# maxjiang93/space_time_pde

Measured on AMD Instinct MI355X. Metric: query-points/sec (fwd+PDE-residual bwd), rb2d 128^3 latent, higher is better.
Workload: dtype f32; 1 GPU; BASELINE configs[1]: latent [1,32,128,128,32], 2^20 query points, RB2 (3 transport + continuity), ImNet nf=32 softplus, L1 losses, backward to ImNet + UNet3d parameters; points=1048576, parallelism=points sharded x1, unet=UNet3d(igres=(32, 128, 128), nf=16, mf=256) fwd+bwd inside the timed step

## Files before the change

include/stpde_hip.h:

```cpp
#ifndef STPDE_HIP_H
#define STPDE_HIP_H

#ifdef __cplusplus
extern "C" {
#endif

#define STPDE_OK 0
#define STPDE_E_BADARG 1
#define STPDE_E_UNSUPPORTED 2
#define STPDE_E_LAUNCH 3

#define STPDE_ACT_TANH 0
#define STPDE_ACT_RELU 1
#define STPDE_ACT_SOFTPLUS 2
#define STPDE_ACT_ELU 3
#define STPDE_ACT_SWISH 4
#define STPDE_ACT_LEAKYRELU 5

#define STPDE_XT 3
#define STPDE_PBAR_SLOTS 64

typedef struct {
  int S1;
  int S2;
  int pair0[6];
  int pair1[6];
  int act;
  float act_param;
  int combo;
  float alpha[6];
} stpde_jet_cfg;

int stpde_version(void);
int stpde_last_error(char* buf, unsigned long n);
#define STPDE_TUNE_CONV3_LDS_OFF 0
#define STPDE_TUNE_CONV3_LDS_MINBLK 1
#define STPDE_TUNE_CONV3_LDS_GX 2
#define STPDE_TUNE_CONV_WGRAD_LDS_GX 3
#define STPDE_TUNE_CONV1_WGRAD_LDS_GX 4
#define STPDE_TUNE_COUNT 5
int stpde_tune(const char* name, int value);
int stpde_trace_enable(int on);
long stpde_trace_read(char* buf, unsigned long n);

typedef struct {
  int P, N, B, n0, n1, n2, C;
  int p_base;
  float lo_c[3], hi_c[3], cube[3];
  float alpha[6];
} stpde_gather_desc;
int stpde_lig_gather(const stpde_gather_desc* d, const float* pts, const float* latent, float* X, float* XR,
                     float* coef, int* cell, float* cw , void* stream);

typedef struct {
  int ntiles, KT, MT, first_hidden;
  stpde_jet_cfg cfg;
  int mfma_bf16;
  int packed;
  int det;
} stpde_layer_desc;
int stpde_jet_layer_fwd(const stpde_layer_desc* d, const float* in_pre, const float* X, const float* Wh_pack,
                        const float* Ws_pack, const float* tanc, const float* W0s_pack, const float* tanc0,
                        float* out_pre, const float* cw ,
                        const void* Wh_pack_bf16, float* z0, void* stream);

int stpde_jet_tail_fwd(const stpde_jet_cfg* cfg, int ntiles, int nf16, const float* in_pre2, const float* X,
                       const float* const* Wh_pack, const float* const* Ws_pack, const float* const* tanc,
                       float* const* out_pre, const float* cw, void* stream);

int stpde_jet_tail_fwd_p(const stpde_jet_cfg* cfg, int ntiles, int nf16, const float* in_pre2, const float* X,
                         const float* const* Wh_pack, const float* const* Ws_pack, const float* const* tanc,
                         float* const* out_pre, const float* cw, int packed, const void* const* Wh16_pack, void* stream);

int stpde_jet_tail_bwd(const stpde_jet_cfg* cfg, int ntiles, int nf16, const float* abar5, const float* const* WhT_pack,
                       const float* const* pre, float* const* abar_out, const float* cw, float* act_param_bar,
                       void* stream);

int stpde_jet_tail_bwd_p(const stpde_jet_cfg* cfg, int ntiles, int nf16, const float* abar5, const float* const* WhT_pack,
                         const float* const* pre, float* const* abar_out, const float* cw, float* act_param_bar, int packed,
                         const void* const* WhT16_pack, void* stream);

int stpde_jet_layer_bwd(const stpde_layer_desc* d, const float* abar_out, const float* WhT_pack, float* in_pre,
                        const float* X, const float* W0s_pack, const float* tanc0, float* abar0, const float* cw,
                        float* act_param_bar, const void* WhT_pack_bf16 ,
                        float* abar0_tan, const float* z0, void* stream);

int stpde_jet_layer_bwd_to(const stpde_layer_desc* d, const float* abar_out, const float* WhT_pack, const float* in_pre,
                           float* abar_in, const float* cw, float* act_param_bar, const void* WhT_pack_bf16, void* stream);

int stpde_jet_wgrad(const stpde_layer_desc* d, int SP, const float* abar_out, const float* in_pre, const float* X,
                    const float* tanc0, float* dW_aug, const float* cw, void* stream);

int stpde_jet_fc1_bwd_supported(const stpde_layer_desc* d);
int stpde_jet_fc1_bwd(const stpde_layer_desc* d, const float* abar1, const void* WhT_pack_bf16, const float* z0,
                      const float* tanc0, const float* cw, const float* X, float* abar0, float* abar0_tan, float* dW_aug,
                      float* act_param_bar, void* stream);

int stpde_lig_reduce_fwd(const stpde_jet_cfg* cfg, int S_mlp, int P, int n_out, const float* out_pre,
                         const float* coef, float* jets, long ldp, void* stream);
int stpde_lig_reduce_bwd(const stpde_jet_cfg* cfg, int S_mlp, int P, int n_out, const float* jets_bar, long ldp,
                         const float* coef, float* abar_out, void* stream);

int stpde_jet_tan0_reduce(int ntiles, int MT, const float* abar0_tan, float* dW_aug, int ldw, int det ,
                          void* stream);

typedef struct {
  int ntiles, nlayers, C, n1, n2;
  int MT[8];
  int SP[8];
  int packed[8];
  int S[8];
} stpde_xbar_desc;
int stpde_lig_xbar_scatter(const stpde_xbar_desc* d, const float* const* abar, const float* const* WsL_pack,
                           const int* cell, float* dlatent, void* stream);
int stpde_lig_xbar_rows(const stpde_xbar_desc* d, const float* const* abar, const float* const* WsL_pack,
                        float* xrows, void* stream);
int stpde_lig_dlatent_reduce(int B, int n0, int n1, int n2, int C, const float* xrows, const int* perm,
                             const int* start, float* dlatent, void* stream);

typedef struct {
  int nlayers;
  int cin, cout, nf16;
  int KT[8], MT[8];
  const float* Wh[8];
  const float* WhT[8];
  const float* Ws[8];
  const float* WsL[8];
  const float* tanc[8];
  const void* Wh16[8];
  const void* WhT16[8];
  int mfma_bf16;
  int packed_mask;
  long dw_off[8];
} stpde_imnet_plan;
typedef struct {
  float* X;
  float* XR;
  float* coef;
  float* cw;
  int* cell;
  float* pre[8];
  float* abar2x;
  float* abar3x;
  float* tan0;
  float* abar0;
  float* abar1x;
  float* abar0x;
  float* xrows;
  int* perm;
  int* start;
  void* sort_tmp;
  unsigned long sort_tmp_bytes;
  float* abar4x;
} stpde_lig_workspace;
#define STPDE_F_STASH 1
#define STPDE_F_VALUE_TILES 2
#define STPDE_F_FUSED_TAIL 4
#define STPDE_F_TAN0_ROWSUM 8
#define STPDE_F_DETERMINISTIC 16
#define STPDE_F_WGRAD 32
#define STPDE_F_WGRAD_FP32 64
#define STPDE_F_PHASE_A 128
#define STPDE_F_PHASE_B 256
#define STPDE_F_NO_FC1_FUSED 512
#define STPDE_F_DET 1024
int stpde_lig_imnet_jet_fwd(const stpde_imnet_plan* plan, const stpde_jet_cfg* cfg_mlp, const stpde_jet_cfg* cfg_out,
                            const stpde_gather_desc* gd, const float* pts, const float* latent,
                            const stpde_lig_workspace* ws, float* jets, long ldp, int flags, void* stream);
int stpde_lig_imnet_jet_bwd(const stpde_imnet_plan* plan, const stpde_jet_cfg* cfg_mlp, const stpde_jet_cfg* cfg_out,
                            const stpde_jet_cfg* cfg_val, const stpde_gather_desc* gd, const stpde_lig_workspace* ws,
                            const float* jets_bar, long ldp, float* dW_flat, float* dlatent, float* act_param_bar,
                            int flags, void* stream);
unsigned long stpde_lig_sort_tmp_bytes(int P, long n_nodes);
int stpde_lig_cell_sort(int P, long n_nodes, const int* cell, int* perm, int* start, void* tmp, unsigned long tmp_bytes,
                        void* stream);

typedef struct {
  int P, N, B, dim, C;
  int n[4];
  float lo_c[4], hi_c[4], cube[4];
} stpde_interp_desc;
int stpde_interp_fwd(const stpde_interp_desc* d, const float* grid, const float* pts, float* out ,
                     float* corner_values , float* weights ,
                     float* x_relative , void* stream);
int stpde_interp_bwd_grid(const stpde_interp_desc* d, const float* pts, const float* out_bar,
                          const float* corner_bar, float* dgrid, void* stream);

typedef struct {
  int B, T, Z, X, Ci, Co, ksize;
  int det;
  int mfma_bf16;
} stpde_conv3d_desc;
#define STPDE_DET_K 6
int stpde_det_finalize(const void* acc, long n, float* out, void* stream);
int stpde_conv3d_fwd(const stpde_conv3d_desc* d, const float* x, const float* w_pack, const float* bias, float* y,
                     void* stream);
int stpde_conv3d_wgrad(const stpde_conv3d_desc* d, const float* x, const float* ybar, float* dW, void* stream);
int stpde_conv3d_wgrad_bias(const stpde_conv3d_desc* d, const float* x, const float* ybar, float* dW, float* dbias,
                            void* stream);

typedef struct {
  stpde_conv3d_desc d;
  const float* x;
  const float* w_pack;
  const float* bias;
  float* y;
  const float* x2;
  const float* w2_pack;
  float* y2;
  const float* wo2_pack;
  const float* bias2;
  const double* in_sums;
  const float* in_gamma;
  const float* in_beta;
  float* in_running_mean;
  float* in_running_var;
  float* in_stat;
  double* out_sums;
  const float* m;
  const float* m_stat;
  const float* m_gamma;
  const float* m_beta;
  float* m_bsum;
  int Ci2, Co2;
  float in_eps, in_momentum;
} stpde_conv3d_fused_args;
int stpde_conv3d_fused(const stpde_conv3d_fused_args* a, int* epilogue_done, void* stream);
int stpde_conv3d_wgrad_onload(const stpde_conv3d_desc* d, const float* x, const float* ybar, float* dW, float* dbias,
                              const float* in_stat, const float* in_gamma, const float* in_beta, void* stream);

#define STPDE_BN_REP 16
typedef struct {
  long N;
  int C, training, relu;
  float eps, momentum;
  int scratch_zeroed;
  int stats_mode;
  int reduce_done;
  int det;
} stpde_bn_desc;
int stpde_bn_fwd(const stpde_bn_desc* d, const float* x, const float* residual, const float* gamma, const float* beta,
                 float* running_mean, float* running_var, float* sums, float* stat, float* y, void* stream);
int stpde_bn_bwd(const stpde_bn_desc* d, const float* x, const float* y, const float* dy, const float* gamma,
                 const float* stat, float* bsum, float* dx, float* dresidual, float* dgamma, float* dbeta, void* stream);

typedef struct {
  int B, T, Z, X, C, ft, fz, fx;
} stpde_resample_desc;
int stpde_resample3d(const stpde_resample_desc* d, int mode, const float* in, const float* aux, float* out,
                     void* stream);

#define STPDE_RES_MAX_INS 192
enum {
  STPDE_RES_JET = 0, STPDE_RES_X, STPDE_RES_CONST, STPDE_RES_ADD, STPDE_RES_SUB, STPDE_RES_MUL, STPDE_RES_DIV,
  STPDE_RES_NEG, STPDE_RES_POWI, STPDE_RES_SIN, STPDE_RES_COS, STPDE_RES_EXP, STPDE_RES_LOG, STPDE_RES_SQRT,
  STPDE_RES_TANH, STPDE_RES_ABS, STPDE_RES_OUT
};
typedef struct {
  int op, a, b;
  float c;
} stpde_res_ins;
int stpde_residual_fwd(const stpde_res_ins* prog_dev, int nins, int n_eq, int n_out, int P, const float* jets,
                       long ld_stream, long ld_channel, const float* x , float* res, void* stream);
int stpde_residual_bwd(const stpde_res_ins* prog_dev, int nins, int n_eq, int n_out, int P, const float* jets,
                       long ld_stream, long ld_channel, const float* x, const float* res_bar, float* jets_bar,
                       void* stream);

#define STPDE_LOSS_L1 0
#define STPDE_LOSS_L2 1
#define STPDE_LOSS_HUBER 2
#define STPDE_LOSS_DET 16
int stpde_loss_sum(int kind, long n, const float* a, const float* b, float* out_sum, void* stream);
int stpde_loss_grad(int kind, long n, const float* a, const float* b, const float* grad_sum_dev, float* grad_a,
                    void* stream);

typedef struct {
  long n;
  float clip, beta1, beta2, eps, weight_decay, step_size, bias2_sqrt;
} stpde_adam_desc;
int stpde_clip_adam(const stpde_adam_desc* d, float* param, const float* grad, float* exp_avg, float* exp_avg_sq,
                    void* stream);
typedef struct {
  float* p;
  const float* g;
  float* m;
  float* v;
  long n;
  float step_size, bias2_sqrt;
} stpde_adam_tensor;
typedef struct {
  int tensor, pad;
  long offset;
} stpde_adam_chunk;
int stpde_clip_adam_multi(const stpde_adam_desc* d, const stpde_adam_tensor* tensors_dev,
                          const stpde_adam_chunk* chunks_dev, int nchunks, int chunk_elems, void* stream);

#ifdef __cplusplus
}
#endif
#endif
```

space_time_pde_amd/csrc/api.cpp:

```cpp
#include <hip/hip_runtime.h>

#include <cstdarg>
#include <cstdio>
#include <cstring>
#include <mutex>
#include <set>
#include <string>

#include "../../include/stpde_hip.h"

static thread_local char g_err[512] = "";

void stpde_set_error(const char* fmt, ...) {
  va_list ap;
  va_start(ap, fmt);
  vsnprintf(g_err, sizeof(g_err), fmt, ap);
  va_end(ap);
}

int stpde_check_launch(const char* what) {
  hipError_t e = hipGetLastError();
  if (e != hipSuccess) {
    stpde_set_error("%s: launch failed: %s", what, hipGetErrorString(e));
    return STPDE_E_LAUNCH;
  }
  return STPDE_OK;
}

extern "C" int stpde_version(void) { return 315; }

#include <atomic>
static const char* const g_tune_names[STPDE_TUNE_COUNT] = {"conv3_lds_off", "conv3_lds_minblk", "conv3_lds_gx", "conv_wgrad_lds_gx",
                                                           "conv1_wgrad_lds_gx"};
static std::atomic<int> g_tune[STPDE_TUNE_COUNT];
int stpde_tune_get(int key) { return (key >= 0 && key < STPDE_TUNE_COUNT) ? g_tune[key].load(std::memory_order_relaxed) : 0; }
extern "C" int stpde_tune(const char* name, int value) {
  if (!name) return -1;
  for (int k = 0; k < STPDE_TUNE_COUNT; ++k)
    if (!strcmp(name, g_tune_names[k])) return g_tune[k].exchange(value);
  stpde_set_error("stpde_tune: unknown key '%s'", name);
  return -1;
}

extern "C" int stpde_last_error(char* buf, unsigned long n) {
  if (!buf || n == 0) return STPDE_E_BADARG;
  strncpy(buf, g_err, n - 1);
  buf[n - 1] = 0;
  return STPDE_OK;
}

int stpde_trace_on = 0;
static std::mutex g_trace_mu;
static std::set<std::string> g_trace;

void stpde_trace_note(const char* launcher, const char* kernel) {
  std::lock_guard<std::mutex> lk(g_trace_mu);
  g_trace.insert(std::string(kernel) + " @ " + launcher);
}

extern "C" int stpde_trace_enable(int on) {
  std::lock_guard<std::mutex> lk(g_trace_mu);
  g_trace.clear();
  stpde_trace_on = on ? 1 : 0;
  return STPDE_OK;
}

extern "C" long stpde_trace_read(char* buf, unsigned long n) {
  std::lock_guard<std::mutex> lk(g_trace_mu);
  std::string all;
  for (const auto& s : g_trace) all += s + "\n";
  if (buf && n > 0) {
    strncpy(buf, all.c_str(), n - 1);
    buf[n - 1] = 0;
  }
  return (long)all.size() + 1;
}
```

space_time_pde_amd/csrc/jet_layer_impl.h:

```cpp
#pragma once
#include <cstdlib>

#include "common.h"

enum { PRO_NONE = 0, PRO_ACT = 1, PRO_L0 = 2 };
enum { EPI_FWD = 0, EPI_ADJ = 1, EPI_ADJ_L0 = 2 };
#ifndef STPDE_ABLATE
#define STPDE_ABLATE 0
#endif

#ifndef STPDE_STAMP
#define STPDE_STAMP 0
#endif
#ifndef STPDE_FWD2_OCC3
#define STPDE_FWD2_OCC3 1
#endif
#ifndef STPDE_FWD2_OCC_N
#define STPDE_FWD2_OCC_N 3
#endif
#ifndef STPDE_EARLY_L0
#define STPDE_EARLY_L0 1
#endif
#ifndef STPDE_EPI_PF
#define STPDE_EPI_PF 1
#endif
#ifndef STPDE_EPI_PF_BF
#define STPDE_EPI_PF_BF 1
#endif
#ifndef STPDE_EPI_PF_DEPTH
#define STPDE_EPI_PF_DEPTH 1
#endif
#ifndef STPDE_EPI_OPF
#define STPDE_EPI_OPF 3
#endif
#ifndef STPDE_X3_STREAM_OUTER
#define STPDE_X3_STREAM_OUTER 1
#endif
#ifndef STPDE_X3_EARLY
#define STPDE_X3_EARLY 0
#endif
#ifndef STPDE_X3_Z0P
#define STPDE_X3_Z0P 0
#endif
#ifndef STPDE_SKIP_FIRST_BAR
#define STPDE_SKIP_FIRST_BAR 1
#endif
#if STPDE_STAMP
#define STPDE_STAMP_B0 8192
static __device__ unsigned long long g_stamp[256 * 8 * 16];
#define STAMP(i)                                                                                          \
  do {                                                                                                    \
    if (blockIdx.x >= STPDE_STAMP_B0 && blockIdx.x < STPDE_STAMP_B0 + 256 && (threadIdx.x & 63) == 0)     \
      g_stamp[((blockIdx.x - STPDE_STAMP_B0) * 8 + (threadIdx.x >> 6)) * 16 + (i)] = __builtin_readcyclecounter(); \
  } while (0)
#else
#define STAMP(i)
#endif

struct LayerArgs {
  const float* Bin;
  const float* Wp;
  const float* X;
  const float* W0s;
  const float* tanc0;
  const float* Wsp;
  const float* tanc;
  float* Out;
  const float* Pre;
  const float* cw;
  const void* Wp16;
  int nsplit;
  float* pbar;
  float* Tan0;
  float* Z0;
  int KT, MT, ntiles;
  int split;
  int pk;
  stpde_jet_cfg cfg;
};

__device__ __forceinline__ f32x4 layer0_block(const float* W0s, int nblk, int blk, int lo, const f32x4* xb) {
  f32x4 part[XT];
#pragma unroll
  for (int xt = 0; xt < XT; ++xt) {
    f32x4 w = ld4x(W0s + ((size_t)xt * nblk + blk) * 256 + lo, xt);
    f32x4 c = f32x4{0.f, 0.f, 0.f, 0.f};
#pragma unroll
    for (int r = 0; r < x_live(xt); ++r) c = mfma4(w[r], xb[xt][r], c);
    part[xt] = c;
  }
  return (part[0] + part[1]) + part[2];
}

template <int S1, int S2, int EPI, int ACT, int PKM = 0>
__device__ __forceinline__ void layer_epilogue(const LayerArgs& a, int tile, int mt, int MT, int lane, f32x4* accm,
                                               const f32x4 (*xbv)[XT], const float* cq, float& pacc,
                                               const f32x4* z0pre = nullptr, const f32x4* prepf = nullptr,
                                               const f32x4* wspf = nullptr, const f32x4* tcpf = nullptr) {
  constexpr int S = 1 + S1 + S2;
  constexpr bool VT = S1 == 0 && S2 > 0;
  const int lo = lane * 4;
  f32x4 (&acc)[1][S] = *reinterpret_cast<f32x4 (*)[1][S]>(accm);
  constexpr int mi = 0;
    if (EPI == EPI_FWD) {
#pragma unroll
      for (int xt = 0; xt < XT; ++xt) {
        f32x4 w = wspf ? wspf[xt] : ld4x(a.Wsp + ((size_t)xt * MT + mt) * 256 + lo, xt);
#pragma unroll
        for (int sv = 0; sv < (VT ? S : 1); ++sv)
#pragma unroll
          for (int r = 0; r < x_live(xt); ++r) acc[mi][sv] = mfma4(w[r], xbv[sv][xt][r], acc[mi][sv]);
      }
      if (S1 == 3) {
#pragma unroll
        for (int d = 0; d < 3; ++d) acc[mi][1 + d] += tcpf ? tcpf[d] : ld4(a.tanc + ((size_t)d * MT + mt) * 256 + lo);
      }
#pragma unroll
      for (int st = 0; st < S; ++st) st_blk(a.Out, (PKM & 2) ? 1 : 0, tile, S, MT, st, mt, lane, acc[mi][st]);
    } else {
      f32x4 pre[S], ab[S];
      if (EPI == EPI_ADJ) {
#pragma unroll
        for (int st = 0; st < S; ++st)
          pre[st] = prepf ? prepf[st] : ld_blk(a.Pre, (PKM & 4) ? 1 : 0, tile, S, MT, st, mt, lane);
      } else {
        pre[0] = z0pre ? *z0pre : ld4(a.Z0 + ((size_t)tile * MT + mt) * 256 + lo);
        if (S1 == 3) {
#pragma unroll
          for (int d = 0; d < 3; ++d) pre[1 + d] = tcpf ? tcpf[d] : ld4(a.tanc0 + ((size_t)d * MT + mt) * 256 + lo);
#pragma unroll
          for (int p = 0; p < S2; ++p) pre[4 + p] = f32x4{0.f, 0.f, 0.f, 0.f};
        }
      }
      act_jet_adj<S1, S2, ACT>(a.cfg, pre, acc[mi], ab, cq);
      if ((ACT == STPDE_ACT_SWISH || (ACT < 0 && a.cfg.act == STPDE_ACT_SWISH)) && a.pbar)
        pacc += swish_beta_adj<S1, S2>(a.cfg, pre, acc[mi], cq);
      constexpr int SO = (EPI == EPI_ADJ) ? S : 1 + S1;
      if (EPI == EPI_ADJ_L0 && S1 == 3 && a.Tan0) {
        st_blk(a.Out, (PKM & 2) ? 2 : 0, tile, 1, MT, 0, mt, lane, ab[0]);
        f32x4 ts[3];
#pragma unroll
        for (int d = 0; d < 3; ++d) ts[d] = row_sum16x4(ab[1 + d]);
        if ((lane & 15) == 15) {
          float* tp = a.Tan0 + ((size_t)tile * MT + mt) * 48 + 4 * (lane >> 4);
#pragma unroll
          for (int d = 0; d < 3; ++d) st4(tp + 16 * d, ts[d]);
        }
      } else {
#pragma unroll
        for (int st = 0; st < SO; ++st) st_blk(a.Out, (PKM & 2) ? 2 : 0, tile, SO, MT, st, mt, lane, ab[st]);
      }
    }
}

template <int EPI, int ACT>
__device__ __forceinline__ void flush_pbar(const LayerArgs& a, float pacc, int lane) {
  if (EPI != EPI_FWD && (ACT == STPDE_ACT_SWISH || (ACT < 0 && a.cfg.act == STPDE_ACT_SWISH)) && a.pbar) {
    const float v = wave_sum(pacc);
    if (lane == 0) atomicAdd(a.pbar + (blockIdx.x % STPDE_PBAR_SLOTS), v);
  }
}

template <int S1, int S2, int MC, int PRO, int EPI, int ACT, bool GUARD>
__global__ __launch_bounds__(256) void k_layer(LayerArgs a) {
  constexpr int S = 1 + S1 + S2;
  const int lane = threadIdx.x & 63;
  const int tile = blockIdx.x * 4 + (threadIdx.x >> 6);
  if (tile >= a.ntiles) return;
  const int KT = a.KT, MT = a.MT;
  const int lo = lane * 4;
  float cq[6];
  load_cq<S2>(a.cw, tile * 2 + ((lane & 15) >> 3), cq);
  float pacc = 0.f;

  constexpr bool VT = S1 == 0 && S2 > 0;
  constexpr int NX = VT ? S : 1;
  f32x4 xb[NX][XT];
  if (PRO == PRO_L0 || EPI == EPI_FWD) {
#pragma unroll
    for (int sv = 0; sv < NX; ++sv)
#pragma unroll
      for (int xt = 0; xt < XT; ++xt) xb[sv][xt] = ld4x(a.X + (((size_t)tile * NX + sv) * XT + xt) * 256 + lo, xt);
  }
  const auto z0r = opt_store_rsrc(a.Z0 ? a.Z0 + (size_t)tile * KT * 256 : nullptr, (unsigned)KT * 1024u);

  for (int mt0 = 0; mt0 < MT; mt0 += MC) {
  f32x4 acc[MC][S];
#pragma unroll
  for (int mi = 0; mi < MC; ++mi)
#pragma unroll
    for (int st = 0; st < S; ++st) acc[mi][st] = f32x4{0.f, 0.f, 0.f, 0.f};
  const float* wp = a.Wp + (size_t)mt0 * 256 + lo;

  auto load_raw = [&](int kt, f32x4* raw) {
    if (PRO == PRO_L0) {
#pragma unroll
      for (int sv = 0; sv < NX; ++sv) raw[sv] = layer0_block(a.W0s, KT, kt, lo, xb[sv]);
      if (!VT) opt_st4(z0r, kt * 1024 + lane * 16, raw[0]);
      if (S1 == 3) {
#pragma unroll
        for (int d = 0; d < 3; ++d) raw[1 + d] = ld4(a.tanc0 + ((size_t)d * KT + kt) * 256 + lo);
#pragma unroll
        for (int p = 0; p < S2; ++p) raw[4 + p] = f32x4{0.f, 0.f, 0.f, 0.f};
      }
    } else {
#pragma unroll
      for (int st = 0; st < S; ++st) raw[st] = ld_blk(a.Bin, 0, tile, S, KT, st, kt, lane);
    }
  };
  auto load_w = [&](int kt, f32x4* w) {
#pragma unroll
    for (int mi = 0; mi < MC; ++mi) {
      const int mi_c = GUARD ? (mt0 + mi < MT ? mi : 0) : mi;
      w[mi] = ld4(wp + ((size_t)kt * MT + mi_c) * 256);
    }
  };

  if (KT > 0) {
    f32x4 Bc[S], wc[MC];
    {
      f32x4 raw[S];
      load_raw(0, raw);
      if (PRO == PRO_NONE) {
#pragma unroll
        for (int st = 0; st < S; ++st) Bc[st] = raw[st];
      } else {
        act_jet_fwd<S1, S2, ACT>(a.cfg, raw, Bc, cq);
      }
      load_w(0, wc);
    }
    for (int kt = 0; kt < KT; ++kt) {
      const int kn = kt + 1 < KT ? kt + 1 : kt;
      f32x4 rawn[S], wn[MC];
      load_raw(kn, rawn);
      load_w(kn, wn);
#pragma unroll
      for (int mi = 0; mi < MC; ++mi)
#pragma unroll
        for (int r = 0; r < 4; ++r)
#pragma unroll
          for (int st = 0; st < S; ++st) acc[mi][st] = mfma4(wc[mi][r], Bc[st][r], acc[mi][st]);
      if (PRO == PRO_NONE) {
#pragma unroll
        for (int st = 0; st < S; ++st) Bc[st] = rawn[st];
      } else {
        act_jet_fwd<S1, S2, ACT>(a.cfg, rawn, Bc, cq);
      }
#pragma unroll
      for (int mi = 0; mi < MC; ++mi) wc[mi] = wn[mi];
    }
  }

#pragma unroll
  for (int mi = 0; mi < MC; ++mi) {
    const int mt = mt0 + mi;
    if (GUARD && mt >= MT) continue;
    layer_epilogue<S1, S2, EPI, ACT>(a, tile, mt, MT, lane, acc[mi], xb, cq, pacc);
  }
  }
  flush_pbar<EPI, ACT>(a, pacc, lane);
}


template <int S1, int S2, int MCg, int PRO, int EPI, int ACT, int NW, bool BF = false, int PK = 1, bool WRING = false,
          int SPL = 1, int PKM = 0>
__global__ __launch_bounds__(64 * NW, ((!BF || SPL == 1) && PRO == PRO_ACT && EPI == EPI_FWD && MCg == 2 && NW == 4 && !WRING && S1 + S2 <= 4 && STPDE_FWD2_OCC3) ? STPDE_FWD2_OCC_N : 2) void k_layer_coop(LayerArgs a) {
  constexpr int S = 1 + S1 + S2, GK = NW * PK;
  static_assert(!WRING || (!BF && GK == 4), "the weight ring is written for 4 k-tiles per group, fp32");
  static_assert(SPL == 1 || (BF && SPL == 3), "operand splitting is a bf16-pipe mode");
  constexpr int BMODE = (PKM & 1) ? (EPI == EPI_FWD ? 1 : 2) : 0;
  __shared__ __attribute__((aligned(16))) float hb[2][GK][S][BF ? 128 * SPL : 256];
  const int lane = threadIdx.x & 63;
  const int wv = threadIdx.x >> 6;
  const int KT = a.KT, MT = a.MT;
  const int lo = lane * 4;
  STAMP(0);
  int tile = blockIdx.x, pass0 = 0, pstep = 1;
  if (a.split > 0) {
    const int L = blockIdx.x, xcd = L & 7, slot = L >> 3;
    pass0 = slot % a.split;
    pstep = a.split;
    tile = (slot / a.split) * 8 + xcd;
    if (tile >= a.ntiles) return;
  }
  float cq[6];
  load_cq<S2>(a.cw, tile * 2 + ((lane & 15) >> 3), cq);
  float pacc = 0.f;

  constexpr bool VT = S1 == 0 && S2 > 0;
  constexpr int NX = VT ? S : 1;
  f32x4 xb[NX][XT];
  if (PRO == PRO_L0 || EPI == EPI_FWD) {
#pragma unroll
    for (int sv = 0; sv < NX; ++sv)
#pragma unroll
      for (int xt = 0; xt < XT; ++xt) xb[sv][xt] = ld4x(a.X + (((size_t)tile * NX + sv) * XT + xt) * 256 + lo, xt);
  }
  const auto z0r = opt_store_rsrc(a.Z0 ? a.Z0 + (size_t)tile * KT * 256 : nullptr, (unsigned)KT * 1024u);

  auto produce = [&](int kt, int buf, int slot) {
    f32x4 raw[S], B[S];
    if (PRO == PRO_L0) {
#pragma unroll
      for (int sv = 0; sv < NX; ++sv) raw[sv] = layer0_block(a.W0s, KT, kt, lo, xb[sv]);
      if (!VT) opt_st4(z0r, kt * 1024 + lane * 16, raw[0]);
      if (S1 == 3) {
#pragma unroll
        for (int d = 0; d < 3; ++d) raw[1 + d] = ld4(a.tanc0 + ((size_t)d * KT + kt) * 256 + lo);
#pragma unroll
        for (int p = 0; p < S2; ++p) raw[4 + p] = f32x4{0.f, 0.f, 0.f, 0.f};
      }
    } else {
#pragma unroll
      for (int st = 0; st < S; ++st) raw[st] = ld_blk(a.Bin, BMODE, tile, S, KT, st, kt, lane);
    }
    if (PRO == PRO_NONE || STPDE_ABLATE == 1) {
#pragma unroll
      for (int st = 0; st < S; ++st) B[st] = raw[st];
    } else {
      act_jet_fwd<S1, S2, ACT>(a.cfg, raw, B, cq);
    }
#pragma unroll
    for (int st = 0; st < S; ++st) {
      if constexpr (BF) {
        f32x4 v = B[st];
#pragma unroll
        for (int t = 0; t < SPL; ++t) {
          const bf16x4 h = to_bf4(v);
          *reinterpret_cast<bf16x4*>(&hb[buf][slot][st][128 * t + lane * 2]) = h;
          if (t + 1 < SPL) v -= bf4_to_f32(h);
        }
      } else {
        st4(&hb[buf][slot][st][lo], B[st]);
      }
    }
  };
  auto store_block = [&](const f32x4* B, int buf, int slot) {
#pragma unroll
    for (int st = 0; st < S; ++st) {
      if constexpr (BF) {
        f32x4 v = B[st];
#pragma unroll
        for (int t = 0; t < SPL; ++t) {
          const bf16x4 h = to_bf4(v);
          *reinterpret_cast<bf16x4*>(&hb[buf][slot][st][128 * t + lane * 2]) = h;
          if (t + 1 < SPL) v -= bf4_to_f32(h);
        }
      } else {
        st4(&hb[buf][slot][st][lo], B[st]);
      }
    }
  };
  auto produce_group = [&](int g, int buf) {
#pragma unroll
    for (int k = 0; k < PK; ++k) produce(GK * g + NW * k + wv, buf, NW * k + wv);
  };

  const int ngroups = KT / GK;
  bool first_pass = true;
  for (int mt0 = (pass0 * NW + wv) * MCg; mt0 < MT; mt0 += pstep * NW * MCg) {
    f32x4 acc[MCg][S];
#pragma unroll
    for (int mi = 0; mi < MCg; ++mi)
#pragma unroll
      for (int st = 0; st < S; ++st) acc[mi][st] = f32x4{0.f, 0.f, 0.f, 0.f};
    constexpr bool Z0P = EPI == EPI_ADJ_L0 && (SPL == 1 || STPDE_X3_Z0P);
    f32x4 z0p[Z0P ? MCg : 1];
    if constexpr (Z0P) {
#pragma unroll
      for (int mi = 0; mi < MCg; ++mi) z0p[mi] = ld4(a.Z0 + ((size_t)tile * MT + mt0 + mi) * 256 + lo);
    }
    const float* wp = a.Wp + (size_t)mt0 * 256 + lo;
    f32x4 wr[WRING ? 4 : 1][MCg];
    if constexpr (WRING) {
#pragma unroll
      for (int q = 0; q < 3; ++q)
#pragma unroll
        for (int mi = 0; mi < MCg; ++mi) wr[q][mi] = ld4(wp + ((size_t)q * MT + mi) * 256);
    }
    if (!STPDE_SKIP_FIRST_BAR || !first_pass) __syncthreads();
    first_pass = false;
    STAMP(1);
    produce_group(0, 0);
    STAMP(2);
    __syncthreads();
    STAMP(3);
    for (int gi = 0; gi < ngroups; ++gi) {
      const int buf = gi & 1;
      const int gnext = gi + 1 < ngroups ? gi + 1 : gi;
      constexpr bool EARLY = PRO == PRO_NONE && (SPL == 1 || STPDE_X3_EARLY);
      constexpr bool EARLY0 = PRO == PRO_L0 && !VT && STPDE_EARLY_L0;
      f32x4 rawn[EARLY ? PK : 1][S];
      if constexpr (EARLY) {
#pragma unroll
        for (int k = 0; k < PK; ++k)
#pragma unroll
          for (int st = 0; st < S; ++st)
            rawn[k][st] = ld_blk(a.Bin, BMODE, tile, S, KT, st, GK * gnext + NW * k + wv, lane);
      }
      f32x4 w0n[EARLY0 ? PK : 1][XT], tcn[EARLY0 ? PK : 1][3];
      if constexpr (EARLY0) {
#pragma unroll
        for (int k = 0; k < PK; ++k) {
          const int kt = GK * gnext + NW * k + wv;
#pragma unroll
          for (int xt = 0; xt < XT; ++xt) w0n[k][xt] = ld4x(a.W0s + ((size_t)xt * KT + kt) * 256 + lo, xt);
          if (S1 == 3) {
#pragma unroll
            for (int d = 0; d < 3; ++d) tcn[k][d] = ld4(a.tanc0 + ((size_t)d * KT + kt) * 256 + lo);
          }
        }
      }
      if constexpr (BF && SPL == 3 && STPDE_X3_STREAM_OUTER) {
        const bf16x8* wp16 = reinterpret_cast<const bf16x8*>(a.Wp16) + (size_t)mt0 * 64 + lane;
        constexpr int PIN = 0x2 | 0x4 | 0x10 | 0x20 | 0x40 | 0x200;
        auto ldB = [&](int q, int st, bf16x8* B) {
#pragma unroll
          for (int t = 0; t < SPL; ++t)
            B[t] = cat8(*reinterpret_cast<const bf16x4*>(&hb[buf][2 * q][st][128 * t + lane * 2]),
                        *reinterpret_cast<const bf16x4*>(&hb[buf][2 * q + 1][st][128 * t + lane * 2]));
        };
        constexpr int TW[6] = {1, 0, 2, 0, 1, 0}, TB[6] = {1, 2, 0, 1, 0, 0};
        bf16x8 Bc[SPL], Bn[SPL];
        ldB(0, 0, Bc);
#pragma unroll
        for (int q = 0; q < GK / 2; ++q) {
          const int kp = GK / 2 * gi + q;
          bf16x8 w8[MCg][SPL];
#pragma unroll
          for (int mi = 0; mi < MCg; ++mi)
#pragma unroll
            for (int t = 0; t < SPL; ++t)
              w8[mi][t] = wp16[(((size_t)t * (KT / 2) + (STPDE_ABLATE == 3 ? q : kp)) * MT + mi) * 64];
#pragma unroll
          for (int st = 0; st < S; ++st) {
            if (st + 1 < S) ldB(q, st + 1, Bn);
            else if (q + 1 < GK / 2) ldB(q + 1, 0, Bn);
            __builtin_amdgcn_sched_barrier(PIN);
#pragma unroll
            for (int c = 0; c < (STPDE_ABLATE == 6 ? 1 : 6); ++c)
#pragma unroll
              for (int mi = 0; mi < MCg; ++mi) acc[mi][st] = mfma_bf(w8[mi][TW[c]], Bc[TB[c]], acc[mi][st]);
            __builtin_amdgcn_sched_barrier(PIN);
#pragma unroll
            for (int t = 0; t < SPL; ++t) Bc[t] = Bn[t];
          }
        }
      } else if constexpr (BF) {
        const bf16x8* wp16 = reinterpret_cast<const bf16x8*>(a.Wp16) + (size_t)mt0 * 64 + lane;
#pragma unroll
        for (int q = 0; q < GK / 2; ++q) {
          const int kp = GK / 2 * gi + q;
          bf16x8 B8[S][SPL], w8[MCg][SPL];
#pragma unroll
          for (int st = 0; st < S; ++st)
#pragma unroll
            for (int t = 0; t < SPL; ++t)
              B8[st][t] = cat8(*reinterpret_cast<const bf16x4*>(&hb[buf][2 * q][st][128 * t + lane * 2]),
                               *reinterpret_cast<const bf16x4*>(&hb[buf][2 * q + 1][st][128 * t + lane * 2]));
#pragma unroll
          for (int mi = 0; mi < MCg; ++mi)
#pragma unroll
            for (int t = 0; t < SPL; ++t)
              w8[mi][t] = wp16[(((size_t)t * (KT / 2) + (STPDE_ABLATE == 3 ? q : kp)) * MT + mi) * 64];
          if constexpr (SPL == 3) {
            constexpr int TW[6] = {1, 0, 2, 0, 1, 0}, TB[6] = {1, 2, 0, 1, 0, 0};
#pragma unroll
            for (int c = 0; c < (STPDE_ABLATE == 6 ? 1 : 6); ++c)
#pragma unroll
              for (int mi = 0; mi < MCg; ++mi)
#pragma unroll
                for (int st = 0; st < S; ++st) acc[mi][st] = mfma_bf(w8[mi][TW[c]], B8[st][TB[c]], acc[mi][st]);
          } else {
#pragma unroll
            for (int mi = 0; mi < MCg; ++mi)
#pragma unroll
              for (int st = 0; st < S; ++st) acc[mi][st] = mfma_bf(w8[mi][0], B8[st][0], acc[mi][st]);
          }
        }
      } else if constexpr (WRING) {
#pragma unroll
        for (int q = 0; q < 4; ++q) {
          const int kt = 4 * gi + q;
          const int ktn = STPDE_ABLATE == 3 ? (q & 1) : (kt + 3 < KT ? kt + 3 : KT - 1);
          f32x4 B[S];
#pragma unroll
          for (int st = 0; st < S; ++st) B[st] = ld4(&hb[buf][q][st][lo]);
#pragma unroll
          for (int mi = 0; mi < MCg; ++mi)
#pragma unroll
            for (int r = 0; r < 4; ++r)
#pragma unroll
              for (int st = 0; st < S; ++st) acc[mi][st] = mfma4(wr[q][mi][r], B[st][r], acc[mi][st]);
#pragma unroll
          for (int mi = 0; mi < MCg; ++mi) wr[(q + 3) & 3][mi] = ld4(wp + ((size_t)ktn * MT + mi) * 256);
        }
      } else {
#pragma unroll
      for (int q = 0; q < GK; ++q) {
        const int kt = GK * gi + q;
        f32x4 B[S], w[MCg];
#pragma unroll
        for (int st = 0; st < S; ++st) B[st] = ld4(&hb[buf][q][st][lo]);
#pragma unroll
        for (int mi = 0; mi < MCg; ++mi) w[mi] = ld4(wp + ((size_t)kt * MT + mi) * 256);
#pragma unroll
        for (int mi = 0; mi < MCg; ++mi)
#pragma unroll
          for (int r = 0; r < 4; ++r)
#pragma unroll
            for (int st = 0; st < S; ++st) acc[mi][st] = mfma4(w[mi][r], B[st][r], acc[mi][st]);
      }
      }
      if constexpr (EARLY) {
#pragma unroll
        for (int k = 0; k < PK; ++k) store_block(rawn[k], buf ^ 1, NW * k + wv);
      } else if constexpr (EARLY0) {
#pragma unroll
        for (int k = 0; k < PK; ++k) {
          const int kt = GK * gnext + NW * k + wv;
          f32x4 raw[S], B[S], part[XT];
#pragma unroll
          for (int xt = 0; xt < XT; ++xt) {
            f32x4 c = f32x4{0.f, 0.f, 0.f, 0.f};
#pragma unroll
            for (int r = 0; r < x_live(xt); ++r) c = mfma4(w0n[k][xt][r], xb[0][xt][r], c);
            part[xt] = c;
          }
          raw[0] = (part[0] + part[1]) + part[2];
          opt_st4(z0r, kt * 1024 + lane * 16, raw[0]);
          if (S1 == 3) {
#pragma unroll
            for (int d = 0; d < 3; ++d) raw[1 + d] = tcn[k][d];
#pragma unroll
            for (int p = 0; p < S2; ++p) raw[4 + p] = f32x4{0.f, 0.f, 0.f, 0.f};
          }
          act_jet_fwd<S1, S2, ACT>(a.cfg, raw, B, cq);
          store_block(B, buf ^ 1, NW * k + wv);
        }
      } else {
        if (STPDE_ABLATE != 5) produce_group(gnext, buf ^ 1);
      }
      if (gi < 8) STAMP(4 + gi);
      if (STPDE_ABLATE != 2) __syncthreads();
    }
    STAMP(12);
    if (STPDE_ABLATE == 4) {
      f32x4 sum = f32x4{0.f, 0.f, 0.f, 0.f};
#pragma unroll
      for (int mi = 0; mi < MCg; ++mi)
#pragma unroll
        for (int st = 0; st < S; ++st) sum += acc[mi][st];
      if (sum[0] == 12345.678f) st4(a.Out + lo, sum);
      continue;
    }
    constexpr bool EPF = EPI == EPI_ADJ && (!BF || (SPL == 1 && STPDE_EPI_PF_BF)) && MCg > 1 && STPDE_EPI_PF;
    if constexpr (EPF) {
      constexpr int PMD = (PKM & 4) ? 1 : 0;
      constexpr int PFD = STPDE_EPI_PF_DEPTH < 1 ? 1 : (STPDE_EPI_PF_DEPTH > MCg ? MCg : STPDE_EPI_PF_DEPTH);
      f32x4 pr[MCg][S];
#pragma unroll
      for (int mi = 0; mi < PFD; ++mi)
#pragma unroll
        for (int st = 0; st < S; ++st) pr[mi][st] = ld_blk(a.Pre, PMD, tile, S, MT, st, mt0 + mi, lane);
#pragma unroll
      for (int mi = 0; mi < MCg; ++mi) {
        if (mi + PFD < MCg) {
#pragma unroll
          for (int st = 0; st < S; ++st) pr[mi + PFD][st] = ld_blk(a.Pre, PMD, tile, S, MT, st, mt0 + mi + PFD, lane);
        }
        __builtin_amdgcn_sched_barrier(0);
        layer_epilogue<S1, S2, EPI, ACT, PKM>(a, tile, mt0 + mi, MT, lane, acc[mi], xb, cq, pacc, nullptr, pr[mi]);
      }
    } else if constexpr (EPI == EPI_ADJ_L0 && S1 == 3 && S <= 5 && (STPDE_EPI_OPF & 1) && (SPL == 1 || (STPDE_EPI_OPF & 4))) {
      if constexpr (SPL == 1) {
        f32x4 z0l[MCg], tcl[MCg][3];
#pragma unroll
        for (int mi = 0; mi < MCg; ++mi) {
          z0l[mi] = Z0P ? z0p[Z0P ? mi : 0] : ld4(a.Z0 + ((size_t)tile * MT + mt0 + mi) * 256 + lo);
#pragma unroll
          for (int d = 0; d < 3; ++d) tcl[mi][d] = ld4(a.tanc0 + ((size_t)d * MT + mt0 + mi) * 256 + lo);
        }
        __builtin_amdgcn_sched_barrier(0);
#pragma unroll
        for (int mi = 0; mi < MCg; ++mi)
          layer_epilogue<S1, S2, EPI, ACT, PKM>(a, tile, mt0 + mi, MT, lane, acc[mi], xb, cq, pacc, &z0l[mi], nullptr, nullptr,
                                                  tcl[mi]);
      } else {
        f32x4 zc, zn, tcc[3], tcn2[3];
        auto fetch = [&](int mt, f32x4& z, f32x4* t) {
          z = ld4(a.Z0 + ((size_t)tile * MT + mt) * 256 + lo);
#pragma unroll
          for (int d = 0; d < 3; ++d) t[d] = ld4(a.tanc0 + ((size_t)d * MT + mt) * 256 + lo);
        };
        __builtin_amdgcn_sched_barrier(0);
        fetch(mt0, zc, tcc);
#pragma unroll
        for (int mi = 0; mi < MCg; ++mi) {
          if (mi + 1 < MCg) fetch(mt0 + mi + 1, zn, tcn2);
          __builtin_amdgcn_sched_barrier(0);
          layer_epilogue<S1, S2, EPI, ACT, PKM>(a, tile, mt0 + mi, MT, lane, acc[mi], xb, cq, pacc, &zc, nullptr, nullptr, tcc);
          __builtin_amdgcn_sched_barrier(0);
          zc = zn;
#pragma unroll
          for (int d = 0; d < 3; ++d) tcc[d] = tcn2[d];
        }
      }
    } else if constexpr (EPI == EPI_FWD && S1 == 3 && !VT && S <= 5 && (STPDE_EPI_OPF & 2) && (SPL == 1 || (STPDE_EPI_OPF & 4))) {
      f32x4 wsc[XT], tcc[3], wsn[XT], tcn2[3];
      auto fetch = [&](int mt, f32x4* w, f32x4* t) {
#pragma unroll
        for (int xt = 0; xt < XT; ++xt) w[xt] = ld4x(a.Wsp + ((size_t)xt * MT + mt) * 256 + lo, xt);
#pragma unroll
        for (int d = 0; d < 3; ++d) t[d] = ld4(a.tanc + ((size_t)d * MT + mt) * 256 + lo);
      };
      if (SPL != 1) __builtin_amdgcn_sched_barrier(0);
      fetch(mt0, wsc, tcc);
#pragma unroll
      for (int mi = 0; mi < MCg; ++mi) {
        if (mi + 1 < MCg) fetch(mt0 + mi + 1, wsn, tcn2);
        __builtin_amdgcn_sched_barrier(0);
        layer_epilogue<S1, S2, EPI, ACT, PKM>(a, tile, mt0 + mi, MT, lane, acc[mi], xb, cq, pacc, nullptr, nullptr, wsc, tcc);
        if (SPL != 1) __builtin_amdgcn_sched_barrier(0);
#pragma unroll
        for (int xt = 0; xt < XT; ++xt) wsc[xt] = wsn[xt];
#pragma unroll
        for (int d = 0; d < 3; ++d) tcc[d] = tcn2[d];
      }
    } else {
#pragma unroll
    for (int mi = 0; mi < MCg; ++mi)
      layer_epilogue<S1, S2, EPI, ACT, PKM>(a, tile, mt0 + mi, MT, lane, acc[mi], xb, cq, pacc,
                                              Z0P ? &z0p[mi] : nullptr);
    }
    STAMP(13);
  }
  flush_pbar<EPI, ACT>(a, pacc, lane);
}

#include "jet_spec_bf16.h"

template <int S1, int S2, int MCg, int PRO, int EPI, int ACT, int NW>
static int launch_layer_coop(const LayerArgs& a0, hipStream_t stream) {
  LayerArgs a = a0;
  if constexpr (PRO == PRO_L0 && EPI == EPI_FWD && NW == 4 && MCg == 4 && S1 == 3 && S2 <= 2) {
    if (a.Wp16 && a.nsplit == 1 && a.MT == 16 && (a.KT == 32 || a.KT == 16))
      return launch_fc1_fwd_spec<S1, S2, ACT>(a, stream);
  }
  if constexpr (PRO == PRO_ACT && EPI == EPI_FWD && NW == 4 && MCg == 2 && S1 == 3 && S2 <= 1) {
    if (a.Wp16 && a.nsplit == 1 && a.pk == 3 && a.KT == 16 && a.MT == 8)
      return launch_fc2_fwd_bf<S1, S2, ACT>(a, stream);
  }
  const int npass = a.MT / (NW * MCg);
  a.split = (PRO != PRO_L0 && npass > 1) ? npass : 0;
  const int nblocks = a.split ? (a.ntiles + 7) / 8 * 8 * a.split : a.ntiles;
  if (a.pk && !(a.Wp16 && a.nsplit == 1)) {
    stpde_set_error("packed layer buffers are a bf16-operand mode (stpde_layer_desc.mfma_bf16 == 1)");
    return STPDE_E_UNSUPPORTED;
  }
  if (a.Wp16 && a.nsplit == 3 && !(S1 + S2 <= 4 && NW == 4)) a.Wp16 = nullptr;
  if (a.Wp16 && a.nsplit == 3) {
    if constexpr (S1 + S2 <= 4 && NW == 4)
      STPDE_LAUNCH((k_layer_coop<S1, S2, MCg, PRO, EPI, ACT, NW, true, 1, false, 3>), dim3(nblocks), dim3(64 * NW), 0, stream, a);
  } else if (a.Wp16) {
    constexpr int PKA = (PRO == PRO_L0 && EPI == EPI_FWD) ? 2 : (PRO == PRO_ACT ? 3 : (EPI == EPI_ADJ ? 7 : 3));
    if (a.pk != 0 && a.pk != PKA) {
      stpde_set_error("packed layer buffers: combination %d not compiled for this kernel kind (expects %d)", a.pk, PKA);
      return STPDE_E_UNSUPPORTED;
    }
    if (a.KT % (2 * NW) == 0) {
      if (a.pk)
        STPDE_LAUNCH((k_layer_coop<S1, S2, MCg, PRO, EPI, ACT, NW, true, 2, false, 1, PKA>), dim3(nblocks), dim3(64 * NW), 0, stream, a);
      else
        STPDE_LAUNCH((k_layer_coop<S1, S2, MCg, PRO, EPI, ACT, NW, true, 2>), dim3(nblocks), dim3(64 * NW), 0, stream, a);
    } else {
      if (a.pk)
        STPDE_LAUNCH((k_layer_coop<S1, S2, MCg, PRO, EPI, ACT, NW, true, 1, false, 1, PKA>), dim3(nblocks), dim3(64 * NW), 0, stream, a);
      else
        STPDE_LAUNCH((k_layer_coop<S1, S2, MCg, PRO, EPI, ACT, NW, true>), dim3(nblocks), dim3(64 * NW), 0, stream, a);
    }
  }
  else {
    if constexpr (NW == 4 && MCg == 4 && S1 + S2 <= 5) {
      STPDE_LAUNCH((k_layer_coop<S1, S2, MCg, PRO, EPI, ACT, NW, false, 1, true>), dim3(nblocks), dim3(64 * NW), 0, stream, a);
    } else {
      STPDE_LAUNCH((k_layer_coop<S1, S2, MCg, PRO, EPI, ACT, NW, false>), dim3(nblocks), dim3(64 * NW), 0, stream, a);
    }
  }
  return stpde_check_launch("k_layer_coop");
}

template <int S1, int S2, int PRO, int EPI, int MCg, int NW>
static int launch_coop_act(const LayerArgs& a, hipStream_t stream) {
  switch (a.cfg.act) {
    case STPDE_ACT_TANH: return launch_layer_coop<S1, S2, MCg, PRO, EPI, STPDE_ACT_TANH, NW>(a, stream);
    case STPDE_ACT_RELU: return launch_layer_coop<S1, S2, MCg, PRO, EPI, STPDE_ACT_RELU, NW>(a, stream);
    case STPDE_ACT_SOFTPLUS: return launch_layer_coop<S1, S2, MCg, PRO, EPI, STPDE_ACT_SOFTPLUS, NW>(a, stream);
    case STPDE_ACT_ELU: return launch_layer_coop<S1, S2, MCg, PRO, EPI, STPDE_ACT_ELU, NW>(a, stream);
    case STPDE_ACT_LEAKYRELU: return launch_layer_coop<S1, S2, MCg, PRO, EPI, STPDE_ACT_LEAKYRELU, NW>(a, stream);
    default: return launch_layer_coop<S1, S2, MCg, PRO, EPI, STPDE_ACT_SWISH, NW>(a, stream);
  }
}

template <int S1, int S2, int MC, int PRO, int EPI, int ACT, bool GUARD>
static int launch_layer(const LayerArgs& a, hipStream_t stream) {
  if (a.pk) {
    stpde_set_error("packed layer buffers need the cooperative bf16 kernels (shape not served by them)");
    return STPDE_E_UNSUPPORTED;
  }
  dim3 grid((a.ntiles + 3) / 4);
  STPDE_LAUNCH((k_layer<S1, S2, MC, PRO, EPI, ACT, GUARD>), grid, dim3(256), 0, stream, a);
  return stpde_check_launch("k_layer");
}

template <int S1, int S2, int PRO, int EPI, int MC>
static int launch_fwd_act_mc(const LayerArgs& a, hipStream_t stream) {
  switch (a.cfg.act) {
    case STPDE_ACT_TANH: return launch_layer<S1, S2, MC, PRO, EPI, STPDE_ACT_TANH, false>(a, stream);
    case STPDE_ACT_RELU: return launch_layer<S1, S2, MC, PRO, EPI, STPDE_ACT_RELU, false>(a, stream);
    case STPDE_ACT_SOFTPLUS: return launch_layer<S1, S2, MC, PRO, EPI, STPDE_ACT_SOFTPLUS, false>(a, stream);
    case STPDE_ACT_ELU: return launch_layer<S1, S2, MC, PRO, EPI, STPDE_ACT_ELU, false>(a, stream);
    case STPDE_ACT_LEAKYRELU: return launch_layer<S1, S2, MC, PRO, EPI, STPDE_ACT_LEAKYRELU, false>(a, stream);
    default: return launch_layer<S1, S2, MC, PRO, EPI, STPDE_ACT_SWISH, false>(a, stream);
  }
}

template <int S1, int S2, int PRO, int EPI>
static int launch_fwd_act(const LayerArgs& a, hipStream_t stream) {
  if (a.MT == 2 && S1 + S2 <= 5) return launch_fwd_act_mc<S1, S2, PRO, EPI, 2>(a, stream);
  if (a.MT == 1 && S1 + S2 <= 5) return launch_fwd_act_mc<S1, S2, PRO, EPI, 1>(a, stream);
  if (a.MT % 4 != 0) return launch_layer<S1, S2, 4, PRO, EPI, -1, true>(a, stream);
  if (a.KT % 4 == 0 && a.KT >= 8 && S1 + S2 <= 5) {
    if (EPI == EPI_FWD) {
      if (a.MT % 16 == 0) return launch_coop_act<S1, S2, PRO, EPI, 4, 4>(a, stream);
      if (a.MT % 8 == 0) return launch_coop_act<S1, S2, PRO, EPI, 2, 4>(a, stream);
    } else {
      if (a.MT % 16 == 0 && S1 + S2 <= 4) return launch_coop_act<S1, S2, PRO, EPI, 4, 4>(a, stream);
      if (a.KT % 8 == 0 && a.MT == 16) return launch_coop_act<S1, S2, PRO, EPI, 2, 8>(a, stream);
      if (a.MT % 8 == 0) return launch_coop_act<S1, S2, PRO, EPI, 2, 4>(a, stream);
    }
  }
  if constexpr (S1 + S2 > 5) {
    if constexpr (S1 + S2 == 7 && EPI == EPI_FWD) {
      if (a.KT % 4 == 0 && a.KT >= 8 && a.MT % 16 == 0) return launch_coop_act<S1, S2, PRO, EPI, 4, 4>(a, stream);
    }
    if (a.KT % 4 == 0 && a.KT >= 8 && a.MT % 8 == 0) return launch_coop_act<S1, S2, PRO, EPI, 2, 4>(a, stream);
  }
  if (PRO != PRO_L0 && S1 + S2 <= 5 && a.MT % 8 == 0) return launch_fwd_act_mc<S1, S2, PRO, EPI, 8>(a, stream);
  return launch_fwd_act_mc<S1, S2, PRO, EPI, 4>(a, stream);
}

template <int S1, int S2>
static int launch_mode(const LayerArgs& a, int mode, hipStream_t stream) {
  if constexpr (S1 == 0 && S2 > 0) {
    if (mode == 0) return launch_fwd_act<S1, S2, PRO_ACT, EPI_FWD>(a, stream);
    if (mode == 1) return launch_fwd_act<S1, S2, PRO_L0, EPI_FWD>(a, stream);
    stpde_set_error("value-tile stream configuration (S1 = 0, S2 > 0) has no backward kernels");
    return STPDE_E_UNSUPPORTED;
  } else {
    switch (mode) {
      case 0: return launch_fwd_act<S1, S2, PRO_ACT, EPI_FWD>(a, stream);
      case 1: return launch_fwd_act<S1, S2, PRO_L0, EPI_FWD>(a, stream);
      case 2: return launch_fwd_act<S1, S2, PRO_NONE, EPI_ADJ>(a, stream);
      default: return launch_fwd_act<S1, S2, PRO_NONE, EPI_ADJ_L0>(a, stream);
    }
  }
}

#define STPDE_DEFINE_LAYER_TU(S1, S2) \
  int stpde_layer_launch_##S1##_##S2(const LayerArgs& a, int mode, hipStream_t stream) { return launch_mode<S1, S2>(a, mode, stream); }

int stpde_layer_launch_0_0(const LayerArgs& a, int mode, hipStream_t stream);
int stpde_layer_launch_3_0(const LayerArgs& a, int mode, hipStream_t stream);
int stpde_layer_launch_3_1(const LayerArgs& a, int mode, hipStream_t stream);
int stpde_layer_launch_3_2(const LayerArgs& a, int mode, hipStream_t stream);
int stpde_layer_launch_3_4(const LayerArgs& a, int mode, hipStream_t stream);
int stpde_layer_launch_3_6(const LayerArgs& a, int mode, hipStream_t stream);
int stpde_layer_launch_0_3(const LayerArgs& a, int mode, hipStream_t stream);
```

Measured before the change: 2.481 million query-points/s.

## Add persistent double-buffered dgrad kernel path for the fc2 adjoint layer

Adds a persistent-block variant of the cooperative adjoint (dgrad) layer for KT=8, MT=16 with three tangent streams. Each block loops over tiles with a grid of twice the CU count. While computing the current tile it prefetches the next tile's B operand into a second LDS buffer via global-to-LDS DMA, and keeps a small register ring of weights. This is meant to hide load latency and cut per-block launch and prologue overhead. It doubles the LDS footprint for that instantiation, which may reduce occupancy, and it adds tuning knobs to disable it or set the grid size.

```diff
diff --git a/include/stpde_hip.h b/include/stpde_hip.h
--- a/include/stpde_hip.h
+++ b/include/stpde_hip.h
@@ -38,7 +38,9 @@
 #define STPDE_TUNE_CONV3_LDS_GX 2
 #define STPDE_TUNE_CONV_WGRAD_LDS_GX 3
 #define STPDE_TUNE_CONV1_WGRAD_LDS_GX 4
-#define STPDE_TUNE_COUNT 5
+#define STPDE_TUNE_FC2_PERSIST_OFF 5
+#define STPDE_TUNE_FC2_PERSIST_GX 6
+#define STPDE_TUNE_COUNT 7
 int stpde_tune(const char* name, int value);
 int stpde_trace_enable(int on);
 long stpde_trace_read(char* buf, unsigned long n);
diff --git a/space_time_pde_amd/csrc/api.cpp b/space_time_pde_amd/csrc/api.cpp
--- a/space_time_pde_amd/csrc/api.cpp
+++ b/space_time_pde_amd/csrc/api.cpp
@@ -31,7 +31,7 @@
 
 #include <atomic>
 static const char* const g_tune_names[STPDE_TUNE_COUNT] = {"conv3_lds_off", "conv3_lds_minblk", "conv3_lds_gx", "conv_wgrad_lds_gx",
-                                                           "conv1_wgrad_lds_gx"};
+                                                           "conv1_wgrad_lds_gx", "fc2_persist_off", "fc2_persist_gx"};
 static std::atomic<int> g_tune[STPDE_TUNE_COUNT];
 int stpde_tune_get(int key) { return (key >= 0 && key < STPDE_TUNE_COUNT) ? g_tune[key].load(std::memory_order_relaxed) : 0; }
 extern "C" int stpde_tune(const char* name, int value) {
diff --git a/space_time_pde_amd/csrc/jet_layer_impl.h b/space_time_pde_amd/csrc/jet_layer_impl.h
--- a/space_time_pde_amd/csrc/jet_layer_impl.h
+++ b/space_time_pde_amd/csrc/jet_layer_impl.h
@@ -77,6 +77,7 @@
   int split;
   int pk;
   stpde_jet_cfg cfg;
+  int persist;
 };
 
 __device__ __forceinline__ f32x4 layer0_block(const float* W0s, int nblk, int blk, int lo, const f32x4* xb) {
@@ -161,6 +162,100 @@
   }
 }
 
+template <int S1, int S2, int ACT>
+__device__ __forceinline__ void layer_dgrad_persist(const LayerArgs& a, float* stg) {
+  constexpr int S = 1 + S1 + S2, KT = 8, MT = 16, MCg = 4, NCH = S * KT, NPW = NCH / 4;
+  static_assert(NCH % 4 == 0 && NPW % 2 == 0 && NPW / 2 <= KT - 3, "DMA pieces: two per k-tile, three k-tiles of cover");
+  constexpr int KL = NPW / 2 - 1;
+  const int lane = threadIdx.x & 63;
+  const int wv = __builtin_amdgcn_readfirstlane(threadIdx.x >> 6);
+  const int lo = lane * 4;
+  const int G = gridDim.x;
+  int tile = blockIdx.x;
+  if (tile >= a.ntiles) return;
+  const int mt0 = wv * MCg;
+  const float* wp = a.Wp + (size_t)mt0 * 256 + lo;
+  auto request = [&](int t, int buf, int p) {
+    const int c = wv + 4 * p;
+    glds16(a.Bin + ((size_t)t * NCH + c) * 256 + lo, stg + (buf * NCH + c) * 256);
+  };
+  f32x4 wr[4][MCg];
+#pragma unroll
+  for (int p = 0; p < NPW; ++p) request(tile, 0, p);
+#pragma unroll
+  for (int q = 0; q < 3; ++q)
+#pragma unroll
+    for (int mi = 0; mi < MCg; ++mi) wr[q][mi] = ld4(wp + ((size_t)q * MT + mi) * 256);
+  asm volatile("s_waitcnt vmcnt(0)" ::: "memory");
+  float pacc = 0.f;
+  for (int buf = 0; tile < a.ntiles; tile += G, buf ^= 1) {
+    const int tn = tile + G < a.ntiles ? tile + G : tile;
+    asm volatile("s_waitcnt lgkmcnt(0)" ::: "memory");
+    __builtin_amdgcn_s_barrier();
+    asm volatile("" ::: "memory");
+    STAMP(1);
+    float cq[6];
+    load_cq<S2>(a.cw, tile * 2 + ((lane & 15) >> 3), cq);
+    f32x4 pr[MCg][S];
+#pragma unroll
+    for (int st = 0; st < S; ++st) pr[0][st] = ld_blk(a.Pre, 0, tile, S, MT, st, mt0, lane);
+    f32x4 acc[MCg][S];
+#pragma unroll
+    for (int mi = 0; mi < MCg; ++mi)
+#pragma unroll
+      for (int st = 0; st < S; ++st) acc[mi][st] = f32x4{0.f, 0.f, 0.f, 0.f};
+    const float* hb = stg + buf * NCH * 256 + lo;
+    constexpr int NODS = 0x1 | 0x2 | 0x4 | 0x8 | 0x10 | 0x20 | 0x40 | 0x400;
+    f32x4 Bc[S], Bn[S];
+#pragma unroll
+    for (int st = 0; st < S; ++st) Bc[st] = ld4(hb + (st * KT) * 256);
+#pragma unroll
+    for (int kt = 0; kt < KT; ++kt) {
+      const int q = kt & 3;
+      __builtin_amdgcn_sched_barrier(NODS);
+      if (kt + 1 < KT) {
+#pragma unroll
+        for (int st = 0; st < S; ++st) Bn[st] = ld4(hb + (st * KT + kt + 1) * 256);
+      }
+#pragma unroll
+      for (int mi = 0; mi < MCg; ++mi)
+#pragma unroll
+        for (int r = 0; r < 4; ++r)
+#pragma unroll
+          for (int st = 0; st < S; ++st) acc[mi][st] = mfma4(wr[q][mi][r], Bc[st][r], acc[mi][st]);
+#pragma unroll
+      for (int st = 0; st < S; ++st) Bc[st] = Bn[st];
+      if (kt + 3 < KT) {
+#pragma unroll
+        for (int mi = 0; mi < MCg; ++mi) wr[(q + 3) & 3][mi] = ld4(wp + ((size_t)(kt + 3) * MT + mi) * 256);
+      }
+      if (kt <= KL) {
+        request(tn, buf ^ 1, 2 * kt);
+        request(tn, buf ^ 1, 2 * kt + 1);
+      }
+    }
+    STAMP(12);
+    __builtin_amdgcn_sched_barrier(0);
+    asm volatile("s_waitcnt vmcnt(0)" ::: "memory");
+#pragma unroll
+    for (int mi = 0; mi < MCg; ++mi) {
+      if (mi + 1 < MCg) {
+#pragma unroll
+        for (int st = 0; st < S; ++st) pr[mi + 1][st] = ld_blk(a.Pre, 0, tile, S, MT, st, mt0 + mi + 1, lane);
+      } else {
+#pragma unroll
+        for (int q = 0; q < 3; ++q)
+#pragma unroll
+          for (int m = 0; m < MCg; ++m) wr[q][m] = ld4(wp + ((size_t)q * MT + m) * 256);
+      }
+      __builtin_amdgcn_sched_barrier(0);
+      layer_epilogue<S1, S2, EPI_ADJ, ACT, 0>(a, tile, mt0 + mi, MT, lane, acc[mi], nullptr, cq, pacc, nullptr, pr[mi]);
+    }
+    STAMP(13);
+  }
+  flush_pbar<EPI_ADJ, ACT>(a, pacc, lane);
+}
+
 template <int S1, int S2, int MC, int PRO, int EPI, int ACT, bool GUARD>
 __global__ __launch_bounds__(256) void k_layer(LayerArgs a) {
   constexpr int S = 1 + S1 + S2;
@@ -269,7 +364,15 @@
   static_assert(!WRING || (!BF && GK == 4), "the weight ring is written for 4 k-tiles per group, fp32");
   static_assert(SPL == 1 || (BF && SPL == 3), "operand splitting is a bf16-pipe mode");
   constexpr int BMODE = (PKM & 1) ? (EPI == EPI_FWD ? 1 : 2) : 0;
-  __shared__ __attribute__((aligned(16))) float hb[2][GK][S][BF ? 128 * SPL : 256];
+  constexpr bool PDG = !BF && SPL == 1 && PKM == 0 && S1 == 3 && S <= 5 && PRO == PRO_NONE && EPI == EPI_ADJ && MCg == 4 &&
+                       NW == 4 && WRING && ACT != STPDE_ACT_SWISH;
+  __shared__ __attribute__((aligned(16))) float hb[2][PDG ? 2 * GK : GK][S][BF ? 128 * SPL : 256];
+  if constexpr (PDG) {
+    if (a.persist) {
+      layer_dgrad_persist<S1, S2, ACT>(a, &hb[0][0][0][0]);
+      return;
+    }
+  }
   const int lane = threadIdx.x & 63;
   const int wv = threadIdx.x >> 6;
   const int KT = a.KT, MT = a.MT;
@@ -682,7 +785,21 @@
   }
   else {
     if constexpr (NW == 4 && MCg == 4 && S1 + S2 <= 5) {
-      STPDE_LAUNCH((k_layer_coop<S1, S2, MCg, PRO, EPI, ACT, NW, false, 1, true>), dim3(nblocks), dim3(64 * NW), 0, stream, a);
+      int grid = nblocks;
+      if constexpr (S1 == 3 && S1 + S2 <= 4 && PRO == PRO_NONE && EPI == EPI_ADJ && ACT != STPDE_ACT_SWISH) {
+        if (a.KT == 8 && a.MT == 16 && !stpde_tune_get(STPDE_TUNE_FC2_PERSIST_OFF)) {
+          int gx = stpde_tune_get(STPDE_TUNE_FC2_PERSIST_GX);
+          if (gx <= 0) {
+            int dev = 0, ncu = 256;
+            (void)hipGetDevice(&dev);
+            (void)hipDeviceGetAttribute(&ncu, hipDeviceAttributeMultiprocessorCount, dev);
+            gx = 2 * ncu;
+          }
+          a.persist = 1;
+          grid = gx < a.ntiles ? gx : a.ntiles;
+        }
+      }
+      STPDE_LAUNCH((k_layer_coop<S1, S2, MCg, PRO, EPI, ACT, NW, false, 1, true>), dim3(grid), dim3(64 * NW), 0, stream, a);
     } else {
       STPDE_LAUNCH((k_layer_coop<S1, S2, MCg, PRO, EPI, ACT, NW, false>), dim3(nblocks), dim3(64 * NW), 0, stream, a);
     }
```

Result: no change. 2.488 million query-points/s (median of 6 runs) (+0.3%).
